# UCSC-VLAA/CLIPA

Hardware: AMD Instinct MI355X
Metric: image-text pairs/sec (whole job), full training step (higher is better)
Workload: dtype bf16

## Files before the change

### clipa_amd/build.py

```python
import hashlib
import os
import subprocess
import sys
from concurrent.futures import ThreadPoolExecutor

HERE = os.path.dirname(os.path.abspath(__file__))
ROOT = os.path.dirname(HERE)
CSRC = os.path.join(HERE, "csrc")
LIBDIR = os.path.join(HERE, "lib")
LIB = os.path.join(LIBDIR, "libclipa_hip.so")
SOURCES = ["gemm_nt.hip", "gemm_nta.hip", "gemm_tn.hip", "gemm_tna.hip", "gemm_tn8.hip", "gemm_f8.hip", "gemm_f8a.hip", "quant.hip", "simce.hip", "layernorm.hip", "attention.hip", "attention_wide.hip", "misc.hip", "augment.hip", "runtime.hip"]
AUDITED = ("gemm_nta.hip", "gemm_tna.hip", "gemm_f8a.hip", "gemm_tn8.hip")
HIPCC = os.environ.get("HIPCC", "/opt/rocm/bin/hipcc")
FLAGS = ["--offload-arch=gfx950", "-O3", "-std=c++17", "-fPIC", "-I", CSRC, "-I", os.path.join(ROOT, "include"),
         "-Wno-unused-result", "-ffp-contract=fast"]


def _digest():
    h = hashlib.sha256()
    for name in sorted(os.listdir(CSRC)) + ["../../include/clipa_hip.h"]:
        path = os.path.join(CSRC, name)
        if os.path.isfile(path):
            with open(path, "rb") as f:
                h.update(name.encode())
                h.update(f.read())
    h.update(" ".join(FLAGS).encode())
    return h.hexdigest()


def build(force=False, verbose=False):
    os.makedirs(LIBDIR, exist_ok=True)
    stamp = os.path.join(LIBDIR, "build.stamp")
    digest = _digest()
    if not force and os.path.exists(LIB) and os.path.exists(stamp) and open(stamp).read().strip() == digest:
        return LIB
    objdir = os.path.join(LIBDIR, "obj")
    os.makedirs(objdir, exist_ok=True)

    def compile_one(src):
        obj = os.path.join(objdir, src.replace(".hip", ".o"))
        cmd = [HIPCC] + FLAGS + ["-c", os.path.join(CSRC, src), "-o", obj]
        if src in AUDITED:
            cmd.append("-save-temps=obj")
        if verbose:
            print(" ".join(cmd), flush=True)
        r = subprocess.run(cmd, capture_output=True, text=True)
        if r.returncode != 0:
            raise RuntimeError(f"hipcc failed for {src}:\n{r.stdout}\n{r.stderr}")
        if verbose and r.stderr.strip():
            print(r.stderr)
        if src in AUDITED:
            asm = os.path.join(objdir, src.replace(".hip", "-hip-amdgcn-amd-amdhsa-gfx950.s"))
            if not os.path.isfile(asm):
                raise RuntimeError(f"ISA audit of {src}: device assembly {asm} not found - this hipcc names its -save-temps "
                                   f"files differently (present: {sorted(f for f in os.listdir(objdir) if f.endswith('.s'))})")
            a = subprocess.run([sys.executable, os.path.join(HERE, "isa_audit.py"), asm], capture_output=True, text=True)
            if a.returncode != 0:
                raise RuntimeError(f"ISA audit of {src} failed (clipa_amd/isa_audit.py):\n{a.stdout[-3000:]}\n{a.stderr[-2000:]}")
        return obj

    with ThreadPoolExecutor(max_workers=len(SOURCES)) as ex:
        objs = list(ex.map(compile_one, SOURCES))
    cmd = [HIPCC, "--offload-arch=gfx950", "-shared", "-fPIC", "-o", LIB] + objs
    r = subprocess.run(cmd, capture_output=True, text=True)
    if r.returncode != 0:
# ... 9 lines not shown
```

### clipa_amd/csrc/attention.hip

```cpp
#include "common.h"
#include <mutex>
#include "clipa_hip.h"
#include "attention_common.h"
#include "internal_hooks.h"

namespace {

template <int NKT, int DH, bool CAUSAL>
__global__ __launch_bounds__((64 * attn_waves<NKT, DH>()), HD<DH>::WGS) void attn_fwd_kernel(AttnArgs pin) {
  constexpr int LP = NKT * 32, RB = HD<DH>::RB, KS = HD<DH>::KS, DT = HD<DH>::DT;
  extern __shared__ __attribute__((aligned(16))) char smem[];
  constexpr int HPW = WGHeads<NKT>::HPW, WPH = attn_waves<NKT, DH>() / HPW;
  const int tid = threadIdx.x, lane = tid & 63;
  const int wave_wg = __builtin_amdgcn_readfirstlane(tid >> 6);
  const int slot = wave_wg / WPH, wave = wave_wg % WPH;
  char* sK = smem + slot * (2 * LP * RB);
  char* sV = sK + LP * RB;
  constexpr bool STAGE = fwd_stages<NKT, DH>();
  char* stage = smem + HPW * (2 * LP * RB) + wave_wg * Stg<DH>::BYTES;
  const int l31 = lane & 31, hi = lane >> 5, q16 = (lane >> 4) & 1, i16 = lane & 15;
  const long nheads = (long)pin.B * pin.H;
  const long head_raw = (long)blockIdx.x * HPW + slot;
  const bool live = head_raw < nheads;
  const long head = live ? head_raw : nheads - 1;
// ... 591 lines not shown
  });
  if (rc_dev[dev]) return rc_dev[dev];
  const dim3 grid((unsigned)((long)a.B * a.H));
  if (BWD) hipLaunchKernelGGL((attn_bwd_long_kernel<DH, CAUSAL>), grid, dim3(256), lds, st, a);
  else hipLaunchKernelGGL((attn_fwd_long_kernel<DH, CAUSAL>), grid, dim3(256), lds, st, a);
  return clipa_check_launch(BWD ? "attn_bwd_long" : "attn_fwd_long");
}
#ifndef CLIPA_ATTN_WIDE
template <bool BWD>
int dispatch_long(const AttnArgs& a, int64_t dh, hipStream_t st) {
  if (dh == 80) return a.causal ? launch_long<80, true, BWD>(a, st) : launch_long<80, false, BWD>(a, st);
  return a.causal ? launch_long<64, true, BWD>(a, st) : launch_long<64, false, BWD>(a, st);
}
#endif

bool wide_head(int64_t dh) { return dh == 88 || dh == 104 || dh == 112; }

int check_args(int64_t B, int64_t H, int64_t L, int64_t dh, int64_t ld_qkv, int64_t ld_o, int causal) {
  if (dh != 64 && dh != 80 && !wide_head(dh)) { clipa_set_error("attention: head dim %ld unsupported (64, 80, 88, 104, 112)", (long)dh); return CLIPA_ERR_ARG; }
  if (wide_head(dh) && causal) { clipa_set_error("attention: head dim %ld is compiled for image towers only (no causal mask)", (long)dh); return CLIPA_ERR_ARG; }
  if (L <= 0 || L > LONG_LMAX) { clipa_set_error("attention: L=%ld outside (0, %d]", (long)L, LONG_LMAX); return CLIPA_ERR_ARG; }
  if (ld_qkv % 8 != 0 || ld_o % 8 != 0) { clipa_set_error("attention: row strides must be multiples of 8 elements"); return CLIPA_ERR_ARG; }
  if (B * H <= 0 || B * H > 0x7fffffffL) { clipa_set_error("attention: bad B*H"); return CLIPA_ERR_ARG; }
  return 0;
}

}

#define ATTN_DISPATCH_DH(fn, DH, a, st)                                     \
  switch (((a).L + 31) / 32) {                                               \
    case 1: return fn<1, DH>(a, st); case 2: return fn<2, DH>(a, st);        \
    case 3: return fn<3, DH>(a, st); case 4: return fn<4, DH>(a, st);        \
    case 5: return fn<5, DH>(a, st); case 6: return fn<6, DH>(a, st);        \
    case 7: return fn<7, DH>(a, st); case 8: return fn<8, DH>(a, st);        \
    default: return fn<9, DH>(a, st);                                        \
  }
#ifdef CLIPA_ATTN_WIDE
template <int NKT, int DH> int wide_fwd(const AttnArgs& a, hipStream_t st) { return launch_fwd_c<NKT, DH, false>(a, st); }
template <int NKT, int DH> int wide_bwd(const AttnArgs& a, hipStream_t st) { return launch_bwd_c<NKT, DH, false>(a, st); }
template <int DH>
int wide_dh(const AttnArgs& a, int bwd, hipStream_t st) {
  if (a.L > 288) return bwd ? launch_long<DH, false, true>(a, st) : launch_long<DH, false, false>(a, st);
  if (bwd) { ATTN_DISPATCH_DH(wide_bwd, DH, a, st) }
  ATTN_DISPATCH_DH(wide_fwd, DH, a, st)
}
extern "C" int clipa_attn_wide_launch(const void* args, int64_t dh, int bwd, void* stream) {
  const AttnArgs& a = *(const AttnArgs*)args;
  if (dh == 88) return wide_dh<88>(a, bwd, (hipStream_t)stream);
  if (dh == 104) return wide_dh<104>(a, bwd, (hipStream_t)stream);
  return wide_dh<112>(a, bwd, (hipStream_t)stream);
}
#else
extern "C" int clipa_attn_wide_launch(const void* args, int64_t dh, int bwd, void* stream);
#ifdef CLIPA_ATTN_PERSISTENT_EXPERIMENT
extern "C" int clipa_attn_bwd1_try(const void* args, int64_t dh, void* stream, int* rc);
extern "C" int clipa_attn_fwd1_try(const void* args, int64_t dh, void* stream, int* rc);
#endif

#define ATTN_DISPATCH(fn, dh, a, st)                 \
  if ((dh) == 80) { ATTN_DISPATCH_DH(fn, 80, a, st) } \
  ATTN_DISPATCH_DH(fn, 64, a, st)

extern "C" int clipa_attention_fwd(const void* q, const void* k, const void* v, void* out, float* stats,
                                   int64_t B, int64_t H, int64_t L, int64_t dh, int64_t ld_qkv, int64_t ld_o,
                                   float scale, int causal, void* stream) {
  if (B * H == 0) return CLIPA_OK;
  if (int rc = check_args(B, H, L, dh, ld_qkv, ld_o, causal)) return rc;
  AttnArgs a = {};
  a.q = (const char*)q; a.k = (const char*)k; a.v = (const char*)v; a.ld_qkv = ld_qkv;
  a.o = (char*)out; a.ld_o = ld_o; a.B = (int)B; a.H = (int)H; a.L = (int)L; a.scale = scale; a.causal = causal;
  a.stats = stats;
  if (wide_head(dh)) return clipa_attn_wide_launch(&a, dh, 0, stream);
  if (L > 288) return dispatch_long<false>(a, dh, (hipStream_t)stream);
#ifdef CLIPA_ATTN_PERSISTENT_EXPERIMENT
  int rc1 = 0;
  if ((clipa_internal_debug_flags() & 524288) && clipa_attn_fwd1_try(&a, dh, stream, &rc1)) return rc1;
#endif
  ATTN_DISPATCH(launch_fwd, dh, a, (hipStream_t)stream)
}

extern "C" int clipa_attention_bwd(const void* q, const void* k, const void* v, const void* out,
                                   const void* d_out, const float* stats, void* dq, void* dk, void* dv, int64_t B, int64_t H,
                                   int64_t L, int64_t dh, int64_t ld_qkv, int64_t ld_o, int64_t ld_dqkv,
                                   float scale, int causal, void* stream) {
  if (B * H == 0) return CLIPA_OK;
  if (int rc = check_args(B, H, L, dh, ld_qkv, ld_o, causal)) return rc;
  if (ld_dqkv % 8 != 0) { clipa_set_error("attention_bwd: ld_dqkv must be a multiple of 8"); return CLIPA_ERR_ARG; }
  if (!stats) { clipa_set_error("attention_bwd: needs the forward's softmax statistics"); return CLIPA_ERR_ARG; }
  AttnArgs a = {};
  a.q = (const char*)q; a.k = (const char*)k; a.v = (const char*)v; a.ld_qkv = ld_qkv;
  a.o_in = (const char*)out; a.d_o = (const char*)d_out; a.ld_o = ld_o;
  a.dq = (char*)dq; a.dk = (char*)dk; a.dv = (char*)dv; a.ld_dqkv = ld_dqkv;
  a.B = (int)B; a.H = (int)H; a.L = (int)L; a.scale = scale; a.causal = causal;
  a.stats = const_cast<float*>(stats);
  if (wide_head(dh)) return clipa_attn_wide_launch(&a, dh, 1, stream);
  if (L > 288) return dispatch_long<true>(a, dh, (hipStream_t)stream);
#ifdef CLIPA_ATTN_PERSISTENT_EXPERIMENT
  int rc1 = 0;
  if ((clipa_internal_debug_flags() & 262144) && clipa_attn_bwd1_try(&a, dh, stream, &rc1)) return rc1;
#endif
  ATTN_DISPATCH(launch_bwd, dh, a, (hipStream_t)stream)
}
namespace {
int varlen_args(const int* seq_start, const int* seq_len, int64_t nseq, int64_t tiles, int64_t dh) {
  if (!seq_start || !seq_len) { clipa_set_error("attention (varlen): seq_start / seq_len missing"); return CLIPA_ERR_ARG; }
  if (tiles < 1 || tiles > 9) { clipa_set_error("attention (varlen): tiles=%ld outside [1, 9] (sequences of up to 288 tokens)", (long)tiles); return CLIPA_ERR_ARG; }
  if (dh != 64 && dh != 80) { clipa_set_error("attention (varlen): head dim %ld unsupported (64 and 80)", (long)dh); return CLIPA_ERR_ARG; }
  (void)nseq;
  return 0;
}
}

extern "C" int clipa_attention_fwd_varlen(const void* q, const void* k, const void* v, void* out, float* stats,
                                          const int32_t* seq_start, const int32_t* seq_len, const int32_t* seq_ids, int64_t nseq,
                                          int64_t tiles, int64_t H, int64_t dh, int64_t ld_qkv, int64_t ld_o, float scale,
                                          int causal, void* stream) {
  if (nseq * H == 0) return CLIPA_OK;
  if (int rc = check_args(nseq, H, 32 * tiles, dh, ld_qkv, ld_o, causal)) return rc;
  if (int rc = varlen_args(seq_start, seq_len, nseq, tiles, dh)) return rc;
  AttnArgs a = {};
  a.q = (const char*)q; a.k = (const char*)k; a.v = (const char*)v; a.ld_qkv = ld_qkv;
  a.o = (char*)out; a.ld_o = ld_o; a.B = (int)nseq; a.H = (int)H; a.L = (int)(32 * tiles); a.scale = scale; a.causal = causal;
  a.stats = stats;
  a.seq_start = seq_start; a.seq_len = seq_len; a.seq_ids = seq_ids;
  ATTN_DISPATCH(launch_fwd, dh, a, (hipStream_t)stream)
}

extern "C" int clipa_attention_bwd_varlen(const void* q, const void* k, const void* v, const void* out, const void* d_out,
                                          const float* stats, void* dq, void* dk, void* dv, const int32_t* seq_start,
                                          const int32_t* seq_len, const int32_t* seq_ids, int64_t nseq, int64_t tiles, int64_t H,
                                          int64_t dh, int64_t ld_qkv, int64_t ld_o, int64_t ld_dqkv, float scale, int causal,
                                          void* stream) {
  if (nseq * H == 0) return CLIPA_OK;
  if (int rc = check_args(nseq, H, 32 * tiles, dh, ld_qkv, ld_o, causal)) return rc;
  if (int rc = varlen_args(seq_start, seq_len, nseq, tiles, dh)) return rc;
  if (ld_dqkv % 8 != 0) { clipa_set_error("attention_bwd (varlen): ld_dqkv must be a multiple of 8"); return CLIPA_ERR_ARG; }
  if (!stats) { clipa_set_error("attention_bwd (varlen): needs the forward's softmax statistics"); return CLIPA_ERR_ARG; }
  AttnArgs a = {};
  a.q = (const char*)q; a.k = (const char*)k; a.v = (const char*)v; a.ld_qkv = ld_qkv;
  a.o_in = (const char*)out; a.d_o = (const char*)d_out; a.ld_o = ld_o;
  a.dq = (char*)dq; a.dk = (char*)dk; a.dv = (char*)dv; a.ld_dqkv = ld_dqkv;
  a.B = (int)nseq; a.H = (int)H; a.L = (int)(32 * tiles); a.scale = scale; a.causal = causal;
  a.stats = const_cast<float*>(stats);
  a.seq_start = seq_start; a.seq_len = seq_len; a.seq_ids = seq_ids;
  ATTN_DISPATCH(launch_bwd, dh, a, (hipStream_t)stream)
}
#endif
```

### clipa_amd/csrc/attention_common.h

```cpp
#pragma once
#include "common.h"

namespace {

struct AttnArgs {
  const char* q; const char* k; const char* v; long ld_qkv;
  char* o; const char* o_in; const char* d_o; long ld_o;
  char* dq; char* dk; char* dv; long ld_dqkv;
  float* stats;
  int B, H, L;
  float scale;
  int causal;
  const int* seq_start; const int* seq_len; const int* seq_ids;
  int abl;
};

template <int DH>
struct HD {
  static constexpr int RB = DH == 64 ? 128 : 256;
  static constexpr int NCH = RB / 16;
  static constexpr int KS = (DH + 15) / 16;
  static constexpr int DT = (DH + 31) / 32;
  static constexpr int WGS = DH == 64 ? 2 : 1;
};
template <int NKT>
struct WGHeads {
  static constexpr int HPW = NKT == 1 ? 4 : (NKT == 2 ? 2 : 1);
  static constexpr int WPH = 4 / HPW;
};
template <int NKT, int DH>
__host__ __device__ constexpr int attn_waves() { return (DH == 80 && NKT >= 5) ? 8 : 4; }

template <int DH>
__device__ __forceinline__ int swz_u(int row) {
  if (DH == 64) return (((row >> 1) & 1) << 2) | ((row >> 2) & 1) | (((row >> 3) & 1) << 1);
  return ((row & 3) << 2) | ((row >> 2) & 3);
}

template <int DH>
__device__ __forceinline__ void dma_image(const __amdgpu_buffer_rsrc_t rs, char* img, int LP, long ld,
                                          int wave, int lane, int nwaves = 4) {
  constexpr int NCH = HD<DH>::NCH, RPP = 1024 / HD<DH>::RB;
  for (int pc = wave; pc < LP / RPP; pc += nwaves) {
    const int row = pc * RPP + lane / NCH;
    const int chunk = (lane & (NCH - 1)) ^ swz_u<DH>(row);
    const unsigned oob = (chunk * 8 >= DH) ? 0x80000000u : 0u;
    __builtin_amdgcn_raw_ptr_buffer_load_lds(rs, LDS_PTR(img + pc * 1024), 16,
                                             (unsigned)(row * ld * 2 + chunk * 16) | oob, 0, 0, 0);
  }
}

template <int DH>
__device__ __forceinline__ bf16x8 frag_direct(const char* img, int rowbase, int l31, int hi, int ks) {
  return *(const bf16x8*)(img + (rowbase + l31) * HD<DH>::RB + (((2 * ks + hi) ^ swz_u<DH>(l31)) << 4));
}

template <int DH>
__device__ __forceinline__ bf16x8 frag_trans(const char* img, int rowbase16, int colbase, int hi, int q16, int i16) {
  constexpr int RB = HD<DH>::RB;
  const int col = colbase + 16 * q16 + 4 * (i16 & 3);
  const int r0 = rowbase16 + 4 * hi + (i16 >> 2);
  const int r1 = r0 + 8;
  const bf16x4 a = __builtin_amdgcn_ds_read_tr16_b64_v4i16(
      (__attribute__((address_space(3))) bf16x4*)(img + r0 * RB + (((col >> 3) ^ swz_u<DH>(r0)) << 4) + (col & 7) * 2));
  const bf16x4 b = __builtin_amdgcn_ds_read_tr16_b64_v4i16(
      (__attribute__((address_space(3))) bf16x4*)(img + r1 * RB + (((col >> 3) ^ swz_u<DH>(r1)) << 4) + (col & 7) * 2));
  bf16x8 f;
// ... 153 lines not shown
```

### clipa_amd/isa_audit.py

```python
#!/usr/bin/env python
import os
import re
import sys


def store_data_races(path, txt, label=r"^(\w[\w.$]*):"):
    def regs(tok):
        m = re.match(r"v\[(\d+):(\d+)\]", tok)
        if m:
            return list(range(int(m.group(1)), int(m.group(2)) + 1))
        m = re.match(r"v(\d+)$", tok)
        return [int(m.group(1))] if m else []
    problems, kernel, prev = [], None, None
    for ln, line in enumerate(txt, 1):
        m = re.match(label, line)
        if m:
            kernel, prev = m.group(1), None
            continue
        if line.startswith(".Lfunc_end"):
            kernel = None
        s = line.strip()
        if kernel is None or not s or s[0] in ";." or s.endswith(":"):
            continue
        code = s.split(";")[0].strip()
# ... 13 lines not shown
    def want(kname):
        m = re.search(r"gemm_nta_kernelILi(\d+)ELi(\d+)E", kname)
        if m:
            pre = int(m.group(2))
            return 32 * (2 if pre in (1, 3) else 1), 32 if pre == 2 else 0
        m = re.search(r"gemm_f8a_kernelILi(\d+)ELi(\d+)ELb([01])ELi(\d+)E", kname)
        pre, outq = (int(m.group(2)), int(m.group(4))) if m else (0, 0)
        return 32 * ((pre == 1) + (outq == 0)), 32 * ((pre in (2, 3)) + (outq != 0))

    def close_kernel():
        if kernel is not None and copies == 0:
            problems.append(f"{path}: {kernel}: no CLIPA_EPI_BEGIN / END markers found (epilogue store count unchecked)")
        if kernel is not None and open_k is not None:
            problems.append(f"{path}: {kernel}: CLIPA_EPI_BEGIN {open_k} without its END")

    for ln, line in enumerate(txt, 1):
        m = re.match(r"^(_ZN\S*gemm_(?:nta|f8a)_kernel\S*):", line)
        if m:
            close_kernel()
            kernel, open_k, count, count8, copies = m.group(1), None, 0, 0, 0
            continue
        if line.startswith(".Lfunc_end"):
            close_kernel()
            kernel = None
        if kernel is None:
            continue
        s = line.strip()
        m = re.match(r";\s*CLIPA_EPI_(BEGIN|END)\s+(\d+)", s)
        if m and m.group(1) == "BEGIN":
            if open_k is not None:
                problems.append(f"{path}:{ln}: {kernel}: nested CLIPA_EPI_BEGIN")
            open_k, count, count8 = m.group(2), 0, 0
        elif m:
            if open_k != m.group(2):
                problems.append(f"{path}:{ln}: {kernel}: CLIPA_EPI_END {m.group(2)} does not close BEGIN {open_k}")
            elif (count, count8) != want(kernel):
                problems.append(f"{path}:{ln}: {kernel}: epilogue copy {open_k} issues {count} buffer_store_dwordx4 + {count8} "
                                f"buffer_store_dwordx2, the tile statement's vmcnt assumes {want(kernel)}")
            open_k, copies = None, copies + 1
        elif open_k is not None:
            code = s.split(";")[0].strip()
            if re.match(r"buffer_store_dwordx4\b", code):
                count += 1
            elif re.match(r"buffer_store_dwordx2\b", code):
                count8 += 1
            elif re.match(r"(buffer|global|flat)_store_", code):
                problems.append(f"{path}:{ln}: {kernel}: store of another width inside the epilogue: `{code}`")
            elif re.match(r"\.LBB\w+:", s) or code.startswith("s_cbranch") or code.startswith("s_branch") or code.startswith("s_setpc"):
                problems.append(f"{path}:{ln}: {kernel}: control flow inside an epilogue copy: `{s}`")
    close_kernel()
    return problems


def audit(path):
    txt = open(path).read().splitlines()
    problems = []
    kernel, in_asm = None, False
    agpr = re.compile(r"(?<![\w.])a\[?\d+")
    for ln, line in enumerate(txt, 1):
        m = re.match(r"^(_ZN\S*gemm_(?:[nt][nt]a|f8a|tn8)_kernel\S*):", line)
        if m:
            kernel = m.group(1)
            in_asm = False
            continue
        if line.startswith(".Lfunc_end") or line.strip().startswith(".end_amdhsa_kernel"):
            kernel = None
        if kernel is None:
            continue
        s = line.strip()
        if s.startswith(";;#ASMSTART"):
            in_asm = True
            continue
        if s.startswith(";;#ASMEND"):
            in_asm = False
            continue
        if in_asm or not s or s.startswith(";") or s.startswith("."):
            continue
        code = s.split(";")[0]
        if "scratch_" in code or "s_scratch" in code:
            problems.append(f"{path}:{ln}: scratch access in {kernel}: {code}")
        if agpr.search(code) and not code.startswith("v_accvgpr_read_b32") :
            problems.append(f"{path}:{ln}: compiler-generated AGPR use in {kernel}: {code}")
        if code.startswith("v_accvgpr_write"):
            problems.append(f"{path}:{ln}: compiler-generated v_accvgpr_write in {kernel}: {code}")
    problems += store_data_races(path, txt, r"^(_ZN\S*gemm_(?:[nt][nt]a|f8a|tn8)_kernel\S*):")
    problems += epilogue_store_counts(path, txt)
    meta = "\n".join(txt)
    for m in re.finditer(r"\.name:\s+(\S*gemm_(?:[nt][nt]a|f8a|tn8)_kernel\S*)\n(.*?)\.wavefront_size", meta, re.S):
        name, body = m.group(1), m.group(2)
        for key in ("private_segment_fixed_size", "vgpr_spill_count"):
            v = re.search(rf"\.{key}:\s+(\d+)", body)
            if v and int(v.group(1)) != 0:
                problems.append(f"{name}: .{key} = {v.group(1)} (must be 0)")
        v = re.search(r"\.vgpr_count:\s+(\d+)", body)
        if v and int(v.group(1)) != 512:
            problems.append(f"{name}: .vgpr_count = {v.group(1)} (expected 512)")
    return problems


if __name__ == "__main__":
    if not os.path.isfile(sys.argv[1]):
        print(f"isa_audit: assembly file {sys.argv[1]} not found (hipcc -save-temps naming changed?)")
        sys.exit(2)
    bad = audit(sys.argv[1])
    for b in bad[:40]:
        print(b)
    print(f"isa_audit: {len(bad)} finding(s)")
    sys.exit(1 if bad else 0)
```

Measured before the change: 2457.

## Add specialised attention backward kernels for dh=64, seven key tiles

Adds a new attention_persist.hip with two backward kernels for non-causal dh=64 heads whose padded length is seven 32-row tiles. One kernel, enabled by default, does one head per block with direct-to-LDS buffer DMA and per-tile waitcnt staging. The other is a persistent kernel, behind a debug flag, that prefetches the next head's K/V and rows while computing dK/dV. Both replace the generic templated backward dispatch and extend the ISA audit with sweep-marker and scratch checks. The cost is hand-written inline assembly with hard-coded vmcnt counts, plus a dependency on L matching the specialised shape.

```diff
diff --git a/clipa_amd/build.py b/clipa_amd/build.py
--- a/clipa_amd/build.py
+++ b/clipa_amd/build.py
@@ -9,8 +9,8 @@
 CSRC = os.path.join(HERE, "csrc")
 LIBDIR = os.path.join(HERE, "lib")
 LIB = os.path.join(LIBDIR, "libclipa_hip.so")
-SOURCES = ["gemm_nt.hip", "gemm_nta.hip", "gemm_tn.hip", "gemm_tna.hip", "gemm_tn8.hip", "gemm_f8.hip", "gemm_f8a.hip", "quant.hip", "simce.hip", "layernorm.hip", "attention.hip", "attention_wide.hip", "misc.hip", "augment.hip", "runtime.hip"]
-AUDITED = ("gemm_nta.hip", "gemm_tna.hip", "gemm_f8a.hip", "gemm_tn8.hip")
+SOURCES = ["gemm_nt.hip", "gemm_nta.hip", "gemm_tn.hip", "gemm_tna.hip", "gemm_tn8.hip", "gemm_f8.hip", "gemm_f8a.hip", "quant.hip", "simce.hip", "layernorm.hip", "attention.hip", "attention_wide.hip", "attention_persist.hip", "misc.hip", "augment.hip", "runtime.hip"]
+AUDITED = ("gemm_nta.hip", "gemm_tna.hip", "gemm_f8a.hip", "gemm_tn8.hip", "attention_persist.hip")
 HIPCC = os.environ.get("HIPCC", "/opt/rocm/bin/hipcc")
 FLAGS = ["--offload-arch=gfx950", "-O3", "-std=c++17", "-fPIC", "-I", CSRC, "-I", os.path.join(ROOT, "include"),
          "-Wno-unused-result", "-ffp-contract=fast"]
diff --git a/clipa_amd/csrc/attention.hip b/clipa_amd/csrc/attention.hip
--- a/clipa_amd/csrc/attention.hip
+++ b/clipa_amd/csrc/attention.hip
@@ -667,10 +667,8 @@
 }
 #else
 extern "C" int clipa_attn_wide_launch(const void* args, int64_t dh, int bwd, void* stream);
-#ifdef CLIPA_ATTN_PERSISTENT_EXPERIMENT
-extern "C" int clipa_attn_bwd1_try(const void* args, int64_t dh, void* stream, int* rc);
-extern "C" int clipa_attn_fwd1_try(const void* args, int64_t dh, void* stream, int* rc);
-#endif
+extern "C" int clipa_attn_bwd_t7_launch(const void* args, void* stream);
+extern "C" int clipa_attn_bwd_persist_launch(const void* args, void* stream);
 
 #define ATTN_DISPATCH(fn, dh, a, st)                 \
   if ((dh) == 80) { ATTN_DISPATCH_DH(fn, 80, a, st) } \
@@ -687,10 +685,6 @@
   a.stats = stats;
   if (wide_head(dh)) return clipa_attn_wide_launch(&a, dh, 0, stream);
   if (L > 288) return dispatch_long<false>(a, dh, (hipStream_t)stream);
-#ifdef CLIPA_ATTN_PERSISTENT_EXPERIMENT
-  int rc1 = 0;
-  if ((clipa_internal_debug_flags() & 524288) && clipa_attn_fwd1_try(&a, dh, stream, &rc1)) return rc1;
-#endif
   ATTN_DISPATCH(launch_fwd, dh, a, (hipStream_t)stream)
 }
 
@@ -710,10 +704,11 @@
   a.stats = const_cast<float*>(stats);
   if (wide_head(dh)) return clipa_attn_wide_launch(&a, dh, 1, stream);
   if (L > 288) return dispatch_long<true>(a, dh, (hipStream_t)stream);
-#ifdef CLIPA_ATTN_PERSISTENT_EXPERIMENT
-  int rc1 = 0;
-  if ((clipa_internal_debug_flags() & 262144) && clipa_attn_bwd1_try(&a, dh, stream, &rc1)) return rc1;
-#endif
+  if (dh == 64 && !causal && (L + 31) / 32 == 7) {
+    const int f = clipa_internal_debug_flags();
+    if (f & 524288) return clipa_attn_bwd_persist_launch(&a, stream);
+    if (!(f & 262144)) return clipa_attn_bwd_t7_launch(&a, stream);
+  }
   ATTN_DISPATCH(launch_bwd, dh, a, (hipStream_t)stream)
 }
 namespace {
diff --git a/clipa_amd/csrc/attention_common.h b/clipa_amd/csrc/attention_common.h
--- a/clipa_amd/csrc/attention_common.h
+++ b/clipa_amd/csrc/attention_common.h
@@ -12,7 +12,6 @@
   float scale;
   int causal;
   const int* seq_start; const int* seq_len; const int* seq_ids;
-  int abl;
 };
 
 template <int DH>
diff --git a/clipa_amd/csrc/attention_persist.hip b/clipa_amd/csrc/attention_persist.hip
--- /dev/null
+++ b/clipa_amd/csrc/attention_persist.hip
@@ -0,0 +1,476 @@
+#include "common.h"
+#include <mutex>
+#include "clipa_hip.h"
+#include "attention_common.h"
+#include "attn_bwd_asm.inc"
+
+namespace {
+
+constexpr int PB_NKT = 7, PB_DH = 64, PB_LP = PB_NKT * 32, PB_RB = 128, PB_KS = 4, PB_DT = 2;
+constexpr int PB_WAVES = 8;
+constexpr int PB_IMG = PB_LP * PB_RB;
+constexpr int PB_SLOT_KV = 0, PB_SLOT_QD = 2 * PB_IMG;
+constexpr int PB_SM = 4 * PB_IMG;
+constexpr int PB_STAGE = PB_SM + 2 * PB_LP * 4;
+constexpr int PB_LDS = PB_STAGE + PB_WAVES * Stg<64>::BYTES;
+static_assert(PB_LDS <= 160 * 1024, "LDS budget");
+static_assert(ATTN_BWD_DMA_PIECES * PB_WAVES == 2 * PB_LP / 8, "DMA pieces");
+
+struct PbHead {
+  size_t hoff, ooff;
+  size_t stat0;
+  long row0;
+  int col0;
+};
+__device__ __forceinline__ PbHead pb_head(const AttnArgs& p, long head) {
+  const int b = (int)(head / p.H), h = (int)(head - (long)b * p.H);
+  const long row0 = (long)b * p.L;
+  PbHead r;
+  r.hoff = ((size_t)row0 * p.ld_qkv + (size_t)h * PB_DH) * 2;
+  r.ooff = ((size_t)row0 * p.ld_o + (size_t)h * PB_DH) * 2;
+  r.stat0 = (size_t)head * p.L;
+  r.row0 = row0;
+  r.col0 = h * PB_DH;
+  return r;
+}
+
+__device__ __forceinline__ u32x4 pb_srd(const void* base, unsigned bytes) {
+  const unsigned long long b = (unsigned long long)base;
+  u32x4 s;
+  s[0] = (unsigned)b;
+  s[1] = (unsigned)(b >> 32) & 0xffffu;
+  s[2] = bytes;
+  s[3] = 0x00020000u;
+  return s;
+}
+
+__device__ __forceinline__ void pb_dma_pair(const char* baseA, long ldA, const char* baseB, long ldB, unsigned nrecA, unsigned nrecB,
+                                            unsigned lds, int wave, int lane) {
+  const u32x4 sa = pb_srd(baseA, nrecA), sb = pb_srd(baseB, nrecB);
+  const u32x4 s3 = wave < 4 ? sa : sb;
+  unsigned v[ATTN_BWD_DMA_PIECES], l[ATTN_BWD_DMA_PIECES];
+#pragma unroll
+  for (int j = 0; j < ATTN_BWD_DMA_PIECES; ++j) {
+    const int pc = wave + PB_WAVES * j;
+    const int img = pc >= PB_LP / 8, piece = pc - img * (PB_LP / 8);
+    const int row = 8 * piece + (lane >> 3);
+    const int chunk = (lane & 7) ^ swz_u<64>(row);
+    v[j] = (unsigned)(row * (img ? ldB : ldA) * 2 + chunk * 16);
+    l[j] = (unsigned)__builtin_amdgcn_readfirstlane((int)(lds + img * PB_IMG + piece * 1024));
+  }
+  asm volatile(ATTN_BWD_DMA_PAIR_ASM
+               :
+               : [v0] "v"(v[0]), [v1] "v"(v[1]), [v2] "v"(v[2]), [v3] "v"(v[3]), [v4] "v"(v[4]), [v5] "v"(v[5]), [v6] "v"(v[6]),
+                 [l0] "s"(l[0]), [l1] "s"(l[1]), [l2] "s"(l[2]), [l3] "s"(l[3]), [l4] "s"(l[4]), [l5] "s"(l[5]), [l6] "s"(l[6]),
+                 [sa] "s"(sa), [sb] "s"(sb), [s3] "s"(s3)
+               : "memory");
+}
+
+struct PbRows {
+  bf16x8 fq[PB_KS], fdo[PB_KS], fo[PB_KS];
+  float2 st;
+};
+__device__ __forceinline__ void pb_load_rows(const AttnArgs& p, const PbHead& hd, int qg, int hi, PbRows& r) {
+  const unsigned nrec = (unsigned)((long)(p.L - 1) * p.ld_qkv * 2 + PB_DH * 2);
+  const unsigned nrec_o = (unsigned)((long)(p.L - 1) * p.ld_o * 2 + PB_DH * 2);
+  load_frags<PB_KS, PB_DH>(make_rsrc(p.q + hd.hoff, nrec), p.ld_qkv, qg, hi, r.fq);
+  load_frags<PB_KS, PB_DH>(make_rsrc(p.d_o + hd.ooff, nrec_o), p.ld_o, qg, hi, r.fdo);
+  load_frags<PB_KS, PB_DH>(make_rsrc(p.o_in + hd.ooff, nrec_o), p.ld_o, qg, hi, r.fo);
+  r.st = *(const float2*)(p.stats + (hd.stat0 + min(qg, p.L - 1)) * 2);
+}
+__device__ __forceinline__ void pb_rows_landed(PbRows& r) {
+#pragma unroll
+  for (int ks = 0; ks < PB_KS; ++ks) asm volatile("" : "+v"(r.fq[ks]), "+v"(r.fdo[ks]), "+v"(r.fo[ks]));
+  asm volatile("" : "+v"(r.st));
+}
+
+__global__ __launch_bounds__(64 * PB_WAVES, 1) void attn_bwd_persist_kernel(AttnArgs p) {
+  constexpr int NKT = PB_NKT, DH = PB_DH, KS = PB_KS, DT = PB_DT;
+  extern __shared__ __attribute__((aligned(16))) char smem[];
+  const int tid = threadIdx.x;
+  const int wave = __builtin_amdgcn_readfirstlane(tid >> 6);
+  const bool tile = wave < NKT;
+  const int t = tile ? wave : NKT - 1;
+  char* img0 = smem + PB_SLOT_KV;
+  char* img1 = img0 + PB_IMG;
+  char* img2 = smem + PB_SLOT_QD;
+  char* img3 = img2 + PB_IMG;
+  float* sM = (float*)(smem + PB_SM);
+  float* sD = sM + PB_LP;
+  char* stage = smem + PB_STAGE + wave * Stg<64>::BYTES;
+  const unsigned lds0 = (unsigned)(size_t)LDS_PTR(smem);
+  const long nheads = (long)p.B * p.H;
+  const float c = p.scale * 1.4426950408889634f;
+  const unsigned nrec = (unsigned)((long)(p.L - 1) * p.ld_qkv * 2 + DH * 2);
+  const unsigned nrec_o = (unsigned)((long)(p.L - 1) * p.ld_o * 2 + DH * 2);
+  int lane = tid & 63;
+  int l31 = lane & 31, hi = lane >> 5, q16 = (lane >> 4) & 1, i16 = lane & 15;
+  int qg = 32 * t + l31;
+
+  long head = blockIdx.x;
+  PbHead hd = pb_head(p, head);
+  PbRows rows;
+  pb_dma_pair(p.k + hd.hoff, p.ld_qkv, p.v + hd.hoff, p.ld_qkv, nrec, nrec, lds0 + PB_SLOT_KV, wave, lane);
+  pb_load_rows(p, hd, qg, hi, rows);
+  asm volatile(ATTN_BWD_DMA_WAIT_ASM ::: "memory");
+  pb_rows_landed(rows);
+
+  for (;;) {
+    asm volatile("" : "+v"(lane));
+    l31 = lane & 31; hi = lane >> 5; q16 = (lane >> 4) & 1; i16 = lane & 15;
+    qg = 32 * t + l31;
+    const long next = head + gridDim.x;
+    const bool more = next < nheads;
+    asm volatile(ATTN_BWD_BARRIER_ASM ::: "memory");
+    pb_dma_pair(p.q + hd.hoff, p.ld_qkv, p.d_o + hd.ooff, p.ld_o, nrec, nrec_o, lds0 + PB_SLOT_QD, wave, lane);
+
+    f32x16 dq[DT];
+    if (tile) {
+      ATTN_BWD_SWEEP_BEGIN(1);
+      float mp = 1e30f;
+      if (qg < p.L) mp = rows.st.x - __builtin_amdgcn_logf(rows.st.y);
+      float Dq = 0.f;
+#pragma unroll
+      for (int ks = 0; ks < KS; ++ks) {
+        float a[8], o8[8];
+        unpack8(__builtin_bit_cast(u32x4, rows.fdo[ks]), a);
+        unpack8(__builtin_bit_cast(u32x4, rows.fo[ks]), o8);
+#pragma unroll
+        for (int i = 0; i < 8; ++i) Dq += a[i] * o8[i];
+      }
+      Dq += __shfl_xor(Dq, 32, 64);
+      if (hi == 0) { sM[qg] = mp; sD[qg] = Dq; }
+      const int lim2 = p.L - 4 * hi;
+#pragma unroll
+      for (int dt = 0; dt < DT; ++dt)
+#pragma unroll
+        for (int r = 0; r < 16; ++r) dq[dt][r] = 0.f;
+#pragma unroll
+      for (int kt = 0; kt < NKT; ++kt) {
+        f32x16 s, dp;
+#pragma unroll
+        for (int r = 0; r < 16; ++r) { s[r] = 0.f; dp[r] = 0.f; }
+#pragma unroll
+        for (int ks = 0; ks < KS; ++ks) {
+          s = __builtin_amdgcn_mfma_f32_32x32x16_bf16(frag_direct<DH>(img0, 32 * kt, l31, hi, ks), rows.fq[ks], s, 0, 0, 0);
+          dp = __builtin_amdgcn_mfma_f32_32x32x16_bf16(frag_direct<DH>(img1, 32 * kt, l31, hi, ks), rows.fdo[ks], dp, 0, 0, 0);
+        }
+        const bool full = kt < NKT - 1;
+        float ds[16];
+#pragma unroll
+        for (int r = 0; r < 16; ++r) {
+          float pe = __builtin_amdgcn_exp2f(fmaf(s[r], c, -mp));
+          if (!full) pe = (32 * kt + 8 * (r >> 2) + (r & 3) < lim2) ? pe : 0.f;
+          ds[r] = pe * (dp[r] - Dq);
+        }
+#pragma unroll
+        for (int s2 = 0; s2 < 2; ++s2) {
+          const bf16x8 dsf = pack_frag(ds + 8 * s2);
+#pragma unroll
+          for (int dt = 0; dt < DT; ++dt)
+            dq[dt] = __builtin_amdgcn_mfma_f32_32x32x16_bf16(frag_trans<DH>(img0, 32 * kt + 16 * s2, 32 * dt, hi, q16, i16), dsf, dq[dt], 0, 0, 0);
+        }
+      }
+      ATTN_BWD_SWEEP_END(1);
+    }
+    asm volatile(ATTN_BWD_DMA_WAIT_ASM ::: "memory");
+    if (tile) store_tile<DH>(stage, p.dq, p.ld_dqkv, hd.row0 + 32 * t, p.L - 32 * t, hd.col0, lane, dq, p.scale);
+    bf16x8 fk[KS], fv[KS];
+#pragma unroll
+    for (int ks = 0; ks < KS; ++ks) {
+      fk[ks] = frag_direct<DH>(img0, 32 * t, l31, hi, ks);
+      fv[ks] = frag_direct<DH>(img1, 32 * t, l31, hi, ks);
+    }
+    asm volatile(ATTN_BWD_BARRIER_ASM ::: "memory");
+
+    PbHead hn = hd;
+    if (more) {
+      hn = pb_head(p, next);
+      pb_dma_pair(p.k + hn.hoff, p.ld_qkv, p.v + hn.hoff, p.ld_qkv, nrec, nrec, lds0 + PB_SLOT_KV, wave, lane);
+      pb_load_rows(p, hn, qg, hi, rows);
+    }
+    f32x16 dk[DT], dv[DT];
+    if (tile) {
+      ATTN_BWD_SWEEP_BEGIN(2);
+#pragma unroll
+      for (int dt = 0; dt < DT; ++dt)
+#pragma unroll
+        for (int r = 0; r < 16; ++r) { dk[dt][r] = 0.f; dv[dt][r] = 0.f; }
+      for (int qt = 0; qt < NKT; ++qt) {
+        f32x16 s, dp;
+#pragma unroll
+        for (int r = 0; r < 16; ++r) { s[r] = 0.f; dp[r] = 0.f; }
+#pragma unroll
+        for (int ks = 0; ks < KS; ++ks) {
+          s = __builtin_amdgcn_mfma_f32_32x32x16_bf16(frag_direct<DH>(img2, 32 * qt, l31, hi, ks), fk[ks], s, 0, 0, 0);
+          dp = __builtin_amdgcn_mfma_f32_32x32x16_bf16(frag_direct<DH>(img3, 32 * qt, l31, hi, ks), fv[ks], dp, 0, 0, 0);
+        }
+        float pr[16], ds[16];
+#pragma unroll
+        for (int rq = 0; rq < 4; ++rq) {
+          const int q0 = 32 * qt + 8 * rq + 4 * hi;
+          const float4 m4 = *(const float4*)(sM + q0);
+          const float4 d4 = *(const float4*)(sD + q0);
+          const float mm[4] = {m4.x, m4.y, m4.z, m4.w};
+          const float dd[4] = {d4.x, d4.y, d4.z, d4.w};
+#pragma unroll
+          for (int e = 0; e < 4; ++e) {
+            const int r = 4 * rq + e;
+            float pe = __builtin_amdgcn_exp2f(fmaf(s[r], c, -mm[e]));
+            pr[r] = pe;
+            ds[r] = pe * (dp[r] - dd[e]);
+          }
+        }
+#pragma unroll
+        for (int s2 = 0; s2 < 2; ++s2) {
+          const bf16x8 pf = pack_frag(pr + 8 * s2);
+          const bf16x8 dsf = pack_frag(ds + 8 * s2);
+#pragma unroll
+          for (int dt = 0; dt < DT; ++dt) {
+            dv[dt] = __builtin_amdgcn_mfma_f32_32x32x16_bf16(frag_trans<DH>(img3, 32 * qt + 16 * s2, 32 * dt, hi, q16, i16), pf, dv[dt], 0, 0, 0);
+            dk[dt] = __builtin_amdgcn_mfma_f32_32x32x16_bf16(frag_trans<DH>(img2, 32 * qt + 16 * s2, 32 * dt, hi, q16, i16), dsf, dk[dt], 0, 0, 0);
+          }
+        }
+      }
+      ATTN_BWD_SWEEP_END(2);
+    }
+    asm volatile(ATTN_BWD_DMA_WAIT_ASM ::: "memory");
+    pb_rows_landed(rows);
+    if (tile) {
+      store_tile<DH>(stage, p.dk, p.ld_dqkv, hd.row0 + 32 * t, p.L - 32 * t, hd.col0, lane, dk, p.scale);
+      store_tile<DH>(stage, p.dv, p.ld_dqkv, hd.row0 + 32 * t, p.L - 32 * t, hd.col0, lane, dv, 1.0f);
+    }
+    if (!more) break;
+    head = next;
+    hd = hn;
+  }
+}
+
+template <bool FIRST>
+__device__ __forceinline__ void t7_key_tile(const AttnArgs& p, const char* img0, const char* img1, const float* sM, const float* sD,
+                                            const bf16x8 (&fk)[PB_KS], const bf16x8 (&fv)[PB_KS], float c, int l31, int hi,
+                                            int q16, int i16, f32x16 (&dk)[PB_DT], f32x16 (&dv)[PB_DT]) {
+  constexpr int NKT = PB_NKT, DH = PB_DH, KS = PB_KS, DT = PB_DT;
+#pragma unroll
+  for (int dt = 0; dt < DT; ++dt)
+#pragma unroll
+    for (int r = 0; r < 16; ++r) { dk[dt][r] = 0.f; dv[dt][r] = 0.f; }
+  if constexpr (FIRST) ATTN_BWD_SWEEP_BEGIN(2);
+#pragma unroll (FIRST ? NKT : 1)
+  for (int qt = 0; qt < NKT; ++qt) {
+    if constexpr (FIRST) {
+      switch (qt) {
+        case 0: asm volatile(ATTN_BWD_TILE_WAIT_ASM_0 ::: "memory"); break;
+        case 1: asm volatile(ATTN_BWD_TILE_WAIT_ASM_1 ::: "memory"); break;
+        case 2: asm volatile(ATTN_BWD_TILE_WAIT_ASM_2 ::: "memory"); break;
+        case 3: asm volatile(ATTN_BWD_TILE_WAIT_ASM_3 ::: "memory"); break;
+        case 4: asm volatile(ATTN_BWD_TILE_WAIT_ASM_4 ::: "memory"); break;
+        case 5: asm volatile(ATTN_BWD_TILE_WAIT_ASM_5 ::: "memory"); break;
+        default: asm volatile(ATTN_BWD_TILE_WAIT_ASM_6 ::: "memory"); break;
+      }
+    }
+    f32x16 s, dp;
+#pragma unroll
+    for (int r = 0; r < 16; ++r) { s[r] = 0.f; dp[r] = 0.f; }
+#pragma unroll
+    for (int ks = 0; ks < KS; ++ks) {
+      s = __builtin_amdgcn_mfma_f32_32x32x16_bf16(frag_direct<DH>(img0, 32 * qt, l31, hi, ks), fk[ks], s, 0, 0, 0);
+      dp = __builtin_amdgcn_mfma_f32_32x32x16_bf16(frag_direct<DH>(img1, 32 * qt, l31, hi, ks), fv[ks], dp, 0, 0, 0);
+    }
+    float pr[16], ds[16];
+#pragma unroll
+    for (int rq = 0; rq < 4; ++rq) {
+      const int q0 = 32 * qt + 8 * rq + 4 * hi;
+      const float4 m4 = *(const float4*)(sM + q0);
+      const float4 d4 = *(const float4*)(sD + q0);
+      const float mm[4] = {m4.x, m4.y, m4.z, m4.w};
+      const float dd[4] = {d4.x, d4.y, d4.z, d4.w};
+#pragma unroll
+      for (int e = 0; e < 4; ++e) {
+        const int r = 4 * rq + e;
+        float pe = __builtin_amdgcn_exp2f(fmaf(s[r], c, -mm[e]));
+        pr[r] = pe;
+        ds[r] = pe * (dp[r] - dd[e]);
+      }
+    }
+#pragma unroll
+    for (int s2 = 0; s2 < 2; ++s2) {
+      const bf16x8 pf = pack_frag(pr + 8 * s2);
+      const bf16x8 dsf = pack_frag(ds + 8 * s2);
+#pragma unroll
+      for (int dt = 0; dt < DT; ++dt) {
+        dv[dt] = __builtin_amdgcn_mfma_f32_32x32x16_bf16(frag_trans<DH>(img1, 32 * qt + 16 * s2, 32 * dt, hi, q16, i16), pf, dv[dt], 0, 0, 0);
+        dk[dt] = __builtin_amdgcn_mfma_f32_32x32x16_bf16(frag_trans<DH>(img0, 32 * qt + 16 * s2, 32 * dt, hi, q16, i16), dsf, dk[dt], 0, 0, 0);
+      }
+    }
+  }
+  if constexpr (FIRST) ATTN_BWD_SWEEP_END(2);
+}
+
+constexpr int T7_LDS = 2 * PB_IMG + 3 * PB_LP * 4 + 4 * Stg<64>::BYTES;
+
+__global__ __launch_bounds__(256, 2) void attn_bwd_t7_kernel(AttnArgs p) {
+  constexpr int NKT = PB_NKT, DH = PB_DH, KS = PB_KS, DT = PB_DT, LP = PB_LP, RB = PB_RB;
+  extern __shared__ __attribute__((aligned(16))) char smem[];
+  const int tid = threadIdx.x, lane = tid & 63;
+  const int wave = __builtin_amdgcn_readfirstlane(tid >> 6);
+  char* img0 = smem;
+  char* img1 = img0 + LP * RB;
+  float* sM = (float*)(img0 + 2 * LP * RB);
+  float* sD = sM + 2 * LP;
+  char* stage = smem + (2 * LP * RB + 3 * LP * 4) + wave * Stg<DH>::BYTES;
+  const int l31 = lane & 31, hi = lane >> 5, q16 = (lane >> 4) & 1, i16 = lane & 15;
+  const long head = blockIdx.x;
+  const PbHead hd = pb_head(p, head);
+  const unsigned nrec = (unsigned)((long)(p.L - 1) * p.ld_qkv * 2 + DH * 2);
+  const unsigned nrec_o = (unsigned)((long)(p.L - 1) * p.ld_o * 2 + DH * 2);
+  const __amdgpu_buffer_rsrc_t rsQ = make_rsrc(p.q + hd.hoff, nrec), rsK = make_rsrc(p.k + hd.hoff, nrec),
+                               rsV = make_rsrc(p.v + hd.hoff, nrec), rsDO = make_rsrc(p.d_o + hd.ooff, nrec_o),
+                               rsO = make_rsrc(p.o_in + hd.ooff, nrec_o);
+  const float c = p.scale * 1.4426950408889634f;
+  const float* stats = p.stats + hd.stat0 * 2;
+
+  dma_image<DH>(rsK, img0, LP, p.ld_qkv, wave, lane, 4);
+  dma_image<DH>(rsV, img1, LP, p.ld_qkv, wave, lane, 4);
+  bf16x8 fq[KS], fdo[KS], fo[KS];
+  load_frags<KS, DH>(rsQ, p.ld_qkv, 32 * wave + l31, hi, fq);
+  load_frags<KS, DH>(rsDO, p.ld_o, 32 * wave + l31, hi, fdo);
+  load_frags<KS, DH>(rsO, p.ld_o, 32 * wave + l31, hi, fo);
+  __builtin_amdgcn_s_waitcnt(0);
+  __syncthreads();
+  for (int qt = wave; qt < NKT; qt += 4) {
+    const int qg = 32 * qt + l31;
+    if (qt != wave) {
+      load_frags<KS, DH>(rsQ, p.ld_qkv, qg, hi, fq);
+      load_frags<KS, DH>(rsDO, p.ld_o, qg, hi, fdo);
+      load_frags<KS, DH>(rsO, p.ld_o, qg, hi, fo);
+    }
+    float mp = 1e30f;
+    if (qg < p.L) {
+      const float2 st = *(const float2*)(stats + qg * 2);
+      mp = st.x - __builtin_amdgcn_logf(st.y);
+    }
+    float Dq = 0.f;
+#pragma unroll
+    for (int ks = 0; ks < KS; ++ks) {
+      float a[8], o8[8];
+      unpack8(__builtin_bit_cast(u32x4, fdo[ks]), a);
+      unpack8(__builtin_bit_cast(u32x4, fo[ks]), o8);
+#pragma unroll
+      for (int i = 0; i < 8; ++i) Dq += a[i] * o8[i];
+    }
+    Dq += __shfl_xor(Dq, 32, 64);
+    if (hi == 0) { sM[qg] = mp; sD[qg] = Dq; }
+    const int lim2 = p.L - 4 * hi;
+    f32x16 dq[DT];
+#pragma unroll
+    for (int dt = 0; dt < DT; ++dt)
+#pragma unroll
+      for (int r = 0; r < 16; ++r) dq[dt][r] = 0.f;
+#pragma unroll
+    for (int kt = 0; kt < NKT; ++kt) {
+      f32x16 s, dp;
+#pragma unroll
+      for (int r = 0; r < 16; ++r) { s[r] = 0.f; dp[r] = 0.f; }
+#pragma unroll
+      for (int ks = 0; ks < KS; ++ks) {
+        s = __builtin_amdgcn_mfma_f32_32x32x16_bf16(frag_direct<DH>(img0, 32 * kt, l31, hi, ks), fq[ks], s, 0, 0, 0);
+        dp = __builtin_amdgcn_mfma_f32_32x32x16_bf16(frag_direct<DH>(img1, 32 * kt, l31, hi, ks), fdo[ks], dp, 0, 0, 0);
+      }
+      const bool full = kt < NKT - 1;
+      float ds[16];
+#pragma unroll
+      for (int r = 0; r < 16; ++r) {
+        float pe = __builtin_amdgcn_exp2f(fmaf(s[r], c, -mp));
+        if (!full) pe = (32 * kt + 8 * (r >> 2) + (r & 3) < lim2) ? pe : 0.f;
+        ds[r] = pe * (dp[r] - Dq);
+      }
+#pragma unroll
+      for (int s2 = 0; s2 < 2; ++s2) {
+        const bf16x8 dsf = pack_frag(ds + 8 * s2);
+#pragma unroll
+        for (int dt = 0; dt < DT; ++dt)
+          dq[dt] = __builtin_amdgcn_mfma_f32_32x32x16_bf16(frag_trans<DH>(img0, 32 * kt + 16 * s2, 32 * dt, hi, q16, i16), dsf, dq[dt], 0, 0, 0);
+      }
+    }
+    store_tile<DH>(stage, p.dq, p.ld_dqkv, hd.row0 + 32 * qt, p.L - 32 * qt, hd.col0, lane, dq, p.scale);
+  }
+  bf16x8 fk[KS], fv[KS];
+#pragma unroll
+  for (int ks = 0; ks < KS; ++ks) {
+    fk[ks] = frag_direct<DH>(img0, 32 * wave, l31, hi, ks);
+    fv[ks] = frag_direct<DH>(img1, 32 * wave, l31, hi, ks);
+  }
+  asm volatile(ATTN_BWD_BARRIER_ASM ::: "memory");
+
+  {
+    const u32x4 sa = pb_srd(p.q + hd.hoff, nrec), sb = pb_srd(p.d_o + hd.ooff, nrec_o);
+    const unsigned la = (unsigned)__builtin_amdgcn_readfirstlane((int)((unsigned)(size_t)LDS_PTR(img0) + wave * 1024));
+    const unsigned lb = la + PB_IMG;
+    unsigned v[ATTN_BWD_DMA_TILED_PIECES];
+#pragma unroll
+    for (int t = 0; t < NKT; ++t) {
+      const int row = 8 * (4 * t + wave) + (lane >> 3);
+      const int chunk = (lane & 7) ^ swz_u<64>(row);
+      v[2 * t] = (unsigned)(row * p.ld_qkv * 2 + chunk * 16);
+      v[2 * t + 1] = (unsigned)(row * p.ld_o * 2 + chunk * 16);
+    }
+    asm volatile(ATTN_BWD_DMA_TILED_ASM
+                 :
+                 : [v0] "v"(v[0]), [v1] "v"(v[1]), [v2] "v"(v[2]), [v3] "v"(v[3]), [v4] "v"(v[4]), [v5] "v"(v[5]), [v6] "v"(v[6]),
+                   [v7] "v"(v[7]), [v8] "v"(v[8]), [v9] "v"(v[9]), [v10] "v"(v[10]), [v11] "v"(v[11]), [v12] "v"(v[12]),
+                   [v13] "v"(v[13]), [la] "s"(la), [lb] "s"(lb), [sa] "s"(sa), [sb] "s"(sb)
+                 : "memory", "scc");
+  }
+  f32x16 dk[DT], dv[DT];
+  t7_key_tile<true>(p, img0, img1, sM, sD, fk, fv, c, l31, hi, q16, i16, dk, dv);
+  store_tile<DH>(stage, p.dk, p.ld_dqkv, hd.row0 + 32 * wave, p.L - 32 * wave, hd.col0, lane, dk, p.scale);
+  store_tile<DH>(stage, p.dv, p.ld_dqkv, hd.row0 + 32 * wave, p.L - 32 * wave, hd.col0, lane, dv, 1.0f);
+  const int kt = wave + 4;
+  if (kt < NKT) {
+    load_frags<KS, DH>(rsK, p.ld_qkv, 32 * kt + l31, hi, fk);
+    load_frags<KS, DH>(rsV, p.ld_qkv, 32 * kt + l31, hi, fv);
+    t7_key_tile<false>(p, img0, img1, sM, sD, fk, fv, c, l31, hi, q16, i16, dk, dv);
+    store_tile<DH>(stage, p.dk, p.ld_dqkv, hd.row0 + 32 * kt, p.L - 32 * kt, hd.col0, lane, dk, p.scale);
+    store_tile<DH>(stage, p.dv, p.ld_dqkv, hd.row0 + 32 * kt, p.L - 32 * kt, hd.col0, lane, dv, 1.0f);
+  }
+}
+
+}
+
+constexpr int PB_MAX_DEVICES = 64;
+
+extern "C" int clipa_attn_bwd_persist_launch(const void* args, void* stream) {
+  const AttnArgs& a = *(const AttnArgs*)args;
+  static std::once_flag once[PB_MAX_DEVICES];
+  static int rc_dev[PB_MAX_DEVICES], cus_dev[PB_MAX_DEVICES];
+  int dev = 0;
+  if (hipGetDevice(&dev) != hipSuccess || dev < 0 || dev >= PB_MAX_DEVICES) { clipa_set_error("attn_bwd_persist: bad device"); return CLIPA_ERR_LAUNCH; }
+  std::call_once(once[dev], [&]() {
+    rc_dev[dev] = 0;
+    hipError_t e = hipFuncSetAttribute((const void*)attn_bwd_persist_kernel, hipFuncAttributeMaxDynamicSharedMemorySize, PB_LDS);
+    if (e == hipSuccess) e = hipDeviceGetAttribute(&cus_dev[dev], hipDeviceAttributeMultiprocessorCount, dev);
+    if (e != hipSuccess || cus_dev[dev] <= 0) { clipa_set_error("attn_bwd_persist attr: %s", hipGetErrorString(e)); rc_dev[dev] = CLIPA_ERR_LAUNCH; }
+  });
+  if (rc_dev[dev]) return rc_dev[dev];
+  const long nheads = (long)a.B * a.H;
+  const unsigned grid = (unsigned)(nheads < cus_dev[dev] ? nheads : cus_dev[dev]);
+  hipLaunchKernelGGL(attn_bwd_persist_kernel, dim3(grid), dim3(64 * PB_WAVES), PB_LDS, (hipStream_t)stream, a);
+  return clipa_check_launch("attn_bwd_persist");
+}
+
+extern "C" int clipa_attn_bwd_t7_launch(const void* args, void* stream) {
+  const AttnArgs& a = *(const AttnArgs*)args;
+  static std::once_flag once[PB_MAX_DEVICES];
+  static int rc_dev[PB_MAX_DEVICES];
+  int dev = 0;
+  if (hipGetDevice(&dev) != hipSuccess || dev < 0 || dev >= PB_MAX_DEVICES) { clipa_set_error("attn_bwd_t7: bad device"); return CLIPA_ERR_LAUNCH; }
+  std::call_once(once[dev], [&]() {
+    const hipError_t e = hipFuncSetAttribute((const void*)attn_bwd_t7_kernel, hipFuncAttributeMaxDynamicSharedMemorySize, T7_LDS);
+    rc_dev[dev] = 0;
+    if (e != hipSuccess) { clipa_set_error("attn_bwd_t7 attr: %s", hipGetErrorString(e)); rc_dev[dev] = CLIPA_ERR_LAUNCH; }
+  });
+  if (rc_dev[dev]) return rc_dev[dev];
+  hipLaunchKernelGGL(attn_bwd_t7_kernel, dim3((unsigned)((long)a.B * a.H)), dim3(256), T7_LDS, (hipStream_t)stream, a);
+  return clipa_check_launch("attn_bwd_t7");
+}
diff --git a/clipa_amd/csrc/attn_bwd_asm.inc b/clipa_amd/csrc/attn_bwd_asm.inc
--- /dev/null
+++ b/clipa_amd/csrc/attn_bwd_asm.inc
@@ -0,0 +1,82 @@
+#pragma once
+
+#define ATTN_BWD_DMA_PIECES 7
+#define ATTN_BWD_DMA_PAIR_ASM \
+  "s_mov_b32 m0, %[l0]\n\t" \
+  "s_nop 0\n\t" \
+  "buffer_load_dwordx4 %[v0], %[sa], 0 offen lds\n\t" \
+  "s_mov_b32 m0, %[l1]\n\t" \
+  "s_nop 0\n\t" \
+  "buffer_load_dwordx4 %[v1], %[sa], 0 offen lds\n\t" \
+  "s_mov_b32 m0, %[l2]\n\t" \
+  "s_nop 0\n\t" \
+  "buffer_load_dwordx4 %[v2], %[sa], 0 offen lds\n\t" \
+  "s_mov_b32 m0, %[l3]\n\t" \
+  "s_nop 0\n\t" \
+  "buffer_load_dwordx4 %[v3], %[s3], 0 offen lds\n\t" \
+  "s_mov_b32 m0, %[l4]\n\t" \
+  "s_nop 0\n\t" \
+  "buffer_load_dwordx4 %[v4], %[sb], 0 offen lds\n\t" \
+  "s_mov_b32 m0, %[l5]\n\t" \
+  "s_nop 0\n\t" \
+  "buffer_load_dwordx4 %[v5], %[sb], 0 offen lds\n\t" \
+  "s_mov_b32 m0, %[l6]\n\t" \
+  "s_nop 0\n\t" \
+  "buffer_load_dwordx4 %[v6], %[sb], 0 offen lds\n\t"
+
+#define ATTN_BWD_DMA_WAIT_ASM "s_waitcnt vmcnt(0)"
+
+#define ATTN_BWD_DMA_TILED_PIECES 14
+#define ATTN_BWD_DMA_TILED_ASM \
+  "s_add_u32 m0, %[la], 0\n\t" \
+  "s_nop 0\n\t" \
+  "buffer_load_dwordx4 %[v0], %[sa], 0 offen lds\n\t" \
+  "s_add_u32 m0, %[lb], 0\n\t" \
+  "s_nop 0\n\t" \
+  "buffer_load_dwordx4 %[v1], %[sb], 0 offen lds\n\t" \
+  "s_add_u32 m0, %[la], 4096\n\t" \
+  "s_nop 0\n\t" \
+  "buffer_load_dwordx4 %[v2], %[sa], 0 offen lds\n\t" \
+  "s_add_u32 m0, %[lb], 4096\n\t" \
+  "s_nop 0\n\t" \
+  "buffer_load_dwordx4 %[v3], %[sb], 0 offen lds\n\t" \
+  "s_add_u32 m0, %[la], 8192\n\t" \
+  "s_nop 0\n\t" \
+  "buffer_load_dwordx4 %[v4], %[sa], 0 offen lds\n\t" \
+  "s_add_u32 m0, %[lb], 8192\n\t" \
+  "s_nop 0\n\t" \
+  "buffer_load_dwordx4 %[v5], %[sb], 0 offen lds\n\t" \
+  "s_add_u32 m0, %[la], 12288\n\t" \
+  "s_nop 0\n\t" \
+  "buffer_load_dwordx4 %[v6], %[sa], 0 offen lds\n\t" \
+  "s_add_u32 m0, %[lb], 12288\n\t" \
+  "s_nop 0\n\t" \
+  "buffer_load_dwordx4 %[v7], %[sb], 0 offen lds\n\t" \
+  "s_add_u32 m0, %[la], 16384\n\t" \
+  "s_nop 0\n\t" \
+  "buffer_load_dwordx4 %[v8], %[sa], 0 offen lds\n\t" \
+  "s_add_u32 m0, %[lb], 16384\n\t" \
+  "s_nop 0\n\t" \
+  "buffer_load_dwordx4 %[v9], %[sb], 0 offen lds\n\t" \
+  "s_add_u32 m0, %[la], 20480\n\t" \
+  "s_nop 0\n\t" \
+  "buffer_load_dwordx4 %[v10], %[sa], 0 offen lds\n\t" \
+  "s_add_u32 m0, %[lb], 20480\n\t" \
+  "s_nop 0\n\t" \
+  "buffer_load_dwordx4 %[v11], %[sb], 0 offen lds\n\t" \
+  "s_add_u32 m0, %[la], 24576\n\t" \
+  "s_nop 0\n\t" \
+  "buffer_load_dwordx4 %[v12], %[sa], 0 offen lds\n\t" \
+  "s_add_u32 m0, %[lb], 24576\n\t" \
+  "s_nop 0\n\t" \
+  "buffer_load_dwordx4 %[v13], %[sb], 0 offen lds\n\t"
+#define ATTN_BWD_TILE_WAIT_ASM_0 "s_waitcnt vmcnt(12)\n\t" "s_barrier\n\t"
+#define ATTN_BWD_TILE_WAIT_ASM_1 "s_waitcnt vmcnt(10)\n\t" "s_barrier\n\t"
+#define ATTN_BWD_TILE_WAIT_ASM_2 "s_waitcnt vmcnt(8)\n\t" "s_barrier\n\t"
+#define ATTN_BWD_TILE_WAIT_ASM_3 "s_waitcnt vmcnt(6)\n\t" "s_barrier\n\t"
+#define ATTN_BWD_TILE_WAIT_ASM_4 "s_waitcnt vmcnt(4)\n\t" "s_barrier\n\t"
+#define ATTN_BWD_TILE_WAIT_ASM_5 "s_waitcnt vmcnt(2)\n\t" "s_barrier\n\t"
+#define ATTN_BWD_TILE_WAIT_ASM_6 "s_waitcnt vmcnt(0)\n\t" "s_barrier\n\t"
+#define ATTN_BWD_BARRIER_ASM "s_waitcnt lgkmcnt(0)\n\ts_barrier"
+#define ATTN_BWD_SWEEP_BEGIN(K) asm volatile("; CLIPA_SWEEP_BEGIN " #K ::: "memory")
+#define ATTN_BWD_SWEEP_END(K) asm volatile("; CLIPA_SWEEP_END " #K ::: "memory")
diff --git a/clipa_amd/isa_audit.py b/clipa_amd/isa_audit.py
--- a/clipa_amd/isa_audit.py
+++ b/clipa_amd/isa_audit.py
@@ -89,6 +89,53 @@
     return problems
 
 
+def attn_persist_audit(path, txt):
+    problems, kernel, open_k, seen, in_asm = [], None, None, set(), False
+
+    def close():
+        want = {"1", "2"} if kernel is not None and "persist" in kernel else {"2"}
+        if kernel is not None and seen != want:
+            problems.append(f"{path}: {kernel}: sweep markers found for {sorted(seen)}, expected {sorted(want)}")
+
+    for ln, line in enumerate(txt, 1):
+        m = re.match(r"^(_ZN\S*attn_bwd_(?:persist|t7)_kernel\S*):", line)
+        if m:
+            close()
+            kernel, open_k, seen, in_asm = m.group(1), None, set(), False
+            continue
+        if line.startswith(".Lfunc_end"):
+            close()
+            kernel = None
+        if kernel is None:
+            continue
+        s = line.strip()
+        m = re.match(r";\s*CLIPA_SWEEP_(BEGIN|END)\s+(\d+)", s)
+        if m:
+            if m.group(1) == "BEGIN":
+                open_k = m.group(2)
+                seen.add(open_k)
+            else:
+                open_k = None
+            continue
+        if s.startswith(";;#ASMSTART"):
+            in_asm = True
+        elif s.startswith(";;#ASMEND"):
+            in_asm = False
+        code = s.split(";")[0].strip()
+        if "scratch_" in code or "s_scratch" in code:
+            problems.append(f"{path}:{ln}: scratch access in {kernel}: {code}")
+        if open_k is not None and not in_asm and re.match(r"s_waitcnt\b.*vmcnt", code):
+            problems.append(f"{path}:{ln}: {kernel}: `{code}` inside sweep {open_k}")
+    close()
+    meta = "\n".join(txt)
+    for m in re.finditer(r"\.name:\s+(\S*attn_bwd_(?:persist|t7)_kernel\S*)\n(.*?)\.wavefront_size", meta, re.S):
+        for key in ("private_segment_fixed_size", "vgpr_spill_count"):
+            v = re.search(rf"\.{key}:\s+(\d+)", m.group(2))
+            if v and int(v.group(1)) != 0:
+                problems.append(f"{m.group(1)}: .{key} = {v.group(1)} (must be 0)")
+    return problems
+
+
 def audit(path):
     txt = open(path).read().splitlines()
     problems = []
@@ -122,6 +169,7 @@
             problems.append(f"{path}:{ln}: compiler-generated v_accvgpr_write in {kernel}: {code}")
     problems += store_data_races(path, txt, r"^(_ZN\S*gemm_(?:[nt][nt]a|f8a|tn8)_kernel\S*):")
     problems += epilogue_store_counts(path, txt)
+    problems += attn_persist_audit(path, txt)
     meta = "\n".join(txt)
     for m in re.finditer(r"\.name:\s+(\S*gemm_(?:[nt][nt]a|f8a|tn8)_kernel\S*)\n(.*?)\.wavefront_size", meta, re.S):
         name, body = m.group(1), m.group(2)
```

New measurement: 2462, median of 6. About the same (+0.2%).
